# zkcrypto/jubjub

Measured on AMD Instinct MI355X. Metric: Jubjub scalar-muls/sec (varbase), higher is better.
Workload: dtype i32x9 (signed 29-bit limbs, v_mad_i64_i32 integer multiply-add)

## Files before the change

jubjub_amd/csrc/jj_field.h:

```cpp
#pragma once
#if !defined(JJ_EXPERIMENTS) && (defined(JJ_MUL_PIN) || defined(JJ_OPAQUE_MODE) || defined(JJ_VB_MINWAVES) || defined(JJ_VB_W) || defined(JJ_VB_PROBE_SHARED_READS) || \
    defined(JJ_FB_THREADS) || defined(JJ_FB_SINGLE_BUFFER) || defined(JJ_FBC_THREADS) || defined(JJ_FBC_SINGLE_BUFFER) || defined(JJ_FBC_PROBE) || \
    defined(JJ_MSM_SORT_UNROLL) || defined(JJ_MSM_P2_THREADS) || defined(JJ_MSM_ACC_MINBLOCKS))
#error "tuning / probe macros (JJ_VB_W, JJ_FB_THREADS, JJ_FBC_PROBE, ...) need -DJJ_EXPERIMENTS: the shipped library is built with the defaults"
#endif
#ifndef JJ_HOST_EMU
#include <hip/hip_runtime.h>
#endif
#include <stdint.h>
#include "jj_constants.h"

namespace jj {

#ifdef JJ_HOST_EMU
#define JJ_DEV inline
extern "C" void jj_emu_overflow(const char* what);
#define JJ_EMU_ACC_DECL __int128 acc_shadow = 0
#define JJ_EMU_ACC_MAD(x, y) do { acc_shadow += (__int128)(x) * (__int128)(y); if (acc_shadow != (__int128)acc) jj_emu_overflow("column accumulator"); } while (0)
#define JJ_EMU_ACC_SHIFT() do { acc_shadow >>= LB; } while (0)
#else
#define JJ_DEV __device__ __forceinline__
#define JJ_EMU_ACC_DECL
#define JJ_EMU_ACC_MAD(x, y)
#define JJ_EMU_ACC_SHIFT()
#endif

typedef int32_t i32;
typedef int64_t i64;

struct Fe {
  u32 l[NL];
};

#ifndef JJ_MUL_PIN
#define JJ_MUL_PIN 1
#endif
#ifndef JJ_OPAQUE_MODE
#define JJ_OPAQUE_MODE 1
#endif
template <class P, int PIN = JJ_MUL_PIN>
struct Field {
  static constexpr u32 PINV = (0u - P::NINV) & LMASK;

  static JJ_DEV Fe one() { Fe r; _Pragma("unroll") for (int i = 0; i < NL; i++) r.l[i] = P::ONE[i]; return r; }
  static JJ_DEV Fe zero() { Fe r; _Pragma("unroll") for (int i = 0; i < NL; i++) r.l[i] = 0; return r; }
  template <int N>
  static JJ_DEV Fe konst(const u32 (&c)[N]) { Fe r; _Pragma("unroll") for (int i = 0; i < NL; i++) r.l[i] = c[i]; return r; }

#ifdef JJ_HOST_EMU
#define JJ_OPAQUE(x) (x)
#else
#if JJ_OPAQUE_MODE == 1
static __device__ __forceinline__ u32 jj_opaque_asm(u32 x) { asm("" : "+v"(x)); return x; }
#define JJ_OPAQUE(x) jj_opaque_asm(x)
#else
#define JJ_OPAQUE(x) ((u32)__builtin_annotation((u32)(x), "jj"))
#endif
#endif
  template <bool SQUARE, bool DOUBLE, bool OPQ = true>
  static JJ_DEV Fe mul_fips(const Fe& a_in, const Fe& b_in) {
    i32 m[NL];
    i32 b2[NL], b4[NL];
    Fe a, b;
    _Pragma("unroll") for (int i = 0; i < NL; i++) {
      if constexpr (OPQ) { a.l[i] = JJ_OPAQUE(a_in.l[i]); b.l[i] = SQUARE ? a.l[i] : JJ_OPAQUE(b_in.l[i]); }
      else { a.l[i] = a_in.l[i]; b.l[i] = SQUARE ? a.l[i] : b_in.l[i]; }
    }
    if constexpr (SQUARE) {
      _Pragma("unroll") for (int i = 0; i < NL; i++) b2[i] = (i32)(a.l[i] << 1);
      if constexpr (DOUBLE) { _Pragma("unroll") for (int i = 0; i < NL; i++) b4[i] = (i32)(a.l[i] << 2); }
    }
    Fe r;
    i64 acc = 0;
    JJ_EMU_ACC_DECL;
#ifdef JJ_HOST_EMU
#define JJ_PIN(x)
#else
#define JJ_PIN(x) do { if constexpr (PIN == 1) x = __builtin_annotation(x, "jj"); } while (0)
#endif
#define JJ_MAD(x, y) do { acc += (i64)(i32)(x) * (i64)(i32)(y); JJ_EMU_ACC_MAD((i32)(x), (i32)(y)); JJ_PIN(acc); } while (0)
    _Pragma("unroll") for (int k = 0; k < 2 * NL - 1; k++) {
      _Pragma("unroll") for (int i = 0; i < NL; i++) {
        const int j = k - i;
        if (j < 0 || j >= NL) continue;
        if constexpr (SQUARE) {
          if (j > i) { if constexpr (DOUBLE) JJ_MAD(a.l[i], b4[j]); else JJ_MAD(a.l[i], b2[j]); }
          else if (j == i) { if constexpr (DOUBLE) JJ_MAD(a.l[i], b2[i]); else JJ_MAD(a.l[i], a.l[i]); }
        } else {
          JJ_MAD(a.l[i], b.l[j]);
        }
      }
      _Pragma("unroll") for (int i = 0; i < NL; i++) {
        const int j = k - i;
        if (i >= k || i >= NL || j < 1 || j >= NL) continue;
        JJ_MAD(m[i], -(i32)P::P[j]);
      }
      if (k < NL) {
        u32 mk;
        if constexpr (PINV == 1u) mk = (u32)acc & LMASK;
        else mk = ((u32)acc * PINV) & LMASK;
        m[k] = (i32)mk;
        if constexpr (P::P[0] != 1u) JJ_MAD(mk, -(i32)P::P[0]);
      } else {
        r.l[k - NL] = (u32)acc & LMASK;
      }
      acc >>= LB;
      JJ_EMU_ACC_SHIFT();
    }
    r.l[NL - 1] = (u32)acc;
#ifdef JJ_HOST_EMU
    if (acc != (i64)(i32)acc) jj_emu_overflow("top limb");
#endif
#undef JJ_MAD
#undef JJ_PIN
    return r;
  }
  static JJ_DEV Fe mul(const Fe& a, const Fe& b) { return mul_fips<false, false>(a, b); }
  static JJ_DEV Fe opaque(const Fe& a) { Fe r; _Pragma("unroll") for (int i = 0; i < NL; i++) r.l[i] = JJ_OPAQUE(a.l[i]); return r; }
  static JJ_DEV Fe mul_hidden(const Fe& a, const Fe& b) { return mul_fips<false, false, false>(a, b); }
  static JJ_DEV Fe sqr_hidden(const Fe& a) { return mul_fips<true, false, false>(a, a); }
  static JJ_DEV Fe sqr(const Fe& a) { return mul_fips<true, false>(a, a); }
  static JJ_DEV Fe sqr2(const Fe& a) { return mul_fips<true, true>(a, a); }

  static JJ_DEV Fe add(const Fe& a, const Fe& b) {
    Fe r; _Pragma("unroll") for (int i = 0; i < NL; i++) r.l[i] = a.l[i] + b.l[i]; return r;
  }
  static JJ_DEV Fe sub(const Fe& a, const Fe& b) {
    Fe r; _Pragma("unroll") for (int i = 0; i < NL; i++) r.l[i] = a.l[i] - b.l[i]; return r;
  }
  static JJ_DEV Fe neg(const Fe& a) {
    Fe r; _Pragma("unroll") for (int i = 0; i < NL; i++) r.l[i] = 0u - a.l[i]; return r;
  }
  static JJ_DEV Fe dbl(const Fe& a) { return add(a, a); }
  static JJ_DEV Fe dbl_sub(const Fe& a, const Fe& b) {
    Fe r; _Pragma("unroll") for (int i = 0; i < NL; i++) r.l[i] = (a.l[i] << 1) - b.l[i]; return r;
  }
  static JJ_DEV Fe cneg(const Fe& a, u32 mask) {
#ifndef JJ_HOST_EMU
    asm("" : "+v"(mask));
#endif
    Fe r; _Pragma("unroll") for (int i = 0; i < NL; i++) r.l[i] = (a.l[i] ^ mask) - mask; return r;
  }
  static JJ_DEV Fe carry(const Fe& a) {
    Fe r;
    r.l[0] = a.l[0] & LMASK;
    _Pragma("unroll") for (int i = 1; i < NL - 1; i++) r.l[i] = (a.l[i] & LMASK) + (u32)((i32)a.l[i - 1] >> LB);
    r.l[NL - 1] = a.l[NL - 1] + (u32)((i32)a.l[NL - 2] >> LB);
    return r;
  }
  static JJ_DEV Fe carry_full(const Fe& a) {
    Fe r; i32 c = 0;
    _Pragma("unroll") for (int i = 0; i < NL - 1; i++) { const i32 t = (i32)a.l[i] + c; r.l[i] = (u32)t & LMASK; c = t >> LB; }
    r.l[NL - 1] = a.l[NL - 1] + (u32)c;
    return r;
  }
  static JJ_DEV Fe select(const Fe& a, const Fe& b, u32 mask) {
#ifndef JJ_HOST_EMU
    asm("" : "+v"(mask));
#endif
    Fe r; _Pragma("unroll") for (int i = 0; i < NL; i++) r.l[i] = (b.l[i] & mask) | (a.l[i] & ~mask); return r;
  }

  static JJ_DEV Fe to_plain(const Fe& a) {
    Fe one_plain; _Pragma("unroll") for (int i = 0; i < NL; i++) one_plain.l[i] = (i == 0);
    const Fe t = mul(a, one_plain);
    const u32 negm = (u32)((i32)t.l[NL - 1] >> 31);
    Fe s; _Pragma("unroll") for (int i = 0; i < NL; i++) s.l[i] = t.l[i] + (P::P[i] & negm);
    return carry_full(s);
  }
  static JJ_DEV bool is_zero(const Fe& a) {
    Fe one_plain; _Pragma("unroll") for (int i = 0; i < NL; i++) one_plain.l[i] = (i == 0);
    const Fe t = mul(a, one_plain);
    u32 o0 = 0, o1 = 0;
    _Pragma("unroll") for (int i = 0; i < NL; i++) { o0 |= t.l[i]; o1 |= t.l[i] ^ P::NEGP_DIGITS[i]; }
    return o0 == 0 || o1 == 0;
  }
  static JJ_DEV bool eq(const Fe& a, const Fe& b) { return is_zero(sub(a, b)); }
  static JJ_DEV bool is_zero_product(const Fe& t) {
    u32 o0 = 0, o1 = 0;
    _Pragma("unroll") for (int i = 0; i < NL; i++) { o0 |= t.l[i]; o1 |= t.l[i] ^ P::NEGP_DIGITS[i]; }
    return o0 == 0 || o1 == 0;
  }
  static JJ_DEV Fe canon_plain_product(const Fe& a) {
    Fe w = a;
    _Pragma("unroll") for (int rep = 0; rep < 2; rep++) {
      const u32 negm = (u32)((i32)w.l[NL - 1] >> 31);
      Fe s; _Pragma("unroll") for (int i = 0; i < NL; i++) s.l[i] = w.l[i] + (P::P[i] & negm);
      w = carry_full(s);
    }
    return w;
  }
  static JJ_DEV Fe plain_one() { Fe r; _Pragma("unroll") for (int i = 0; i < NL; i++) r.l[i] = (i == 0); return r; }
  static JJ_DEV Fe canon(const Fe& a) {
    Fe w = mul(a, one());
    _Pragma("unroll") for (int rep = 0; rep < 2; rep++) {
      const u32 negm = (u32)((i32)w.l[NL - 1] >> 31);
      Fe s; _Pragma("unroll") for (int i = 0; i < NL; i++) s.l[i] = w.l[i] + (P::P[i] & negm);
      w = carry_full(s);
    }
    return w;
  }

  static JJ_DEV Fe unpack(const u32 (&w)[8]) {
    Fe r;
    _Pragma("unroll") for (int i = 0; i < NL; i++) {
      const int bit = LB * i, wi = bit >> 5, sh = bit & 31;
      u32 v = w[wi] >> sh;
      if (sh > 32 - LB && wi + 1 < 8) v |= w[wi + 1] << (32 - sh);
      r.l[i] = v & LMASK;
    }
    return r;
  }
  static JJ_DEV void pack(u32 (&w)[8], const Fe& a) {
    _Pragma("unroll") for (int wi = 0; wi < 8; wi++) {
      const int bit = 32 * wi, li = bit / LB, sh = bit % LB;
      u32 v = a.l[li] >> sh;
      const int got = LB - sh;
      if (got < 32 && li + 1 < NL) v |= a.l[li + 1] << got;
      if (got + LB < 32 && li + 2 < NL) v |= a.l[li + 2] << (got + LB);
      w[wi] = v;
    }
  }
  static JJ_DEV Fe from_words(const u32 (&w)[8]) { return mul(unpack(w), konst(P::R2)); }
  static JJ_DEV Fe from_words_checked(const u32 (&w)[8], bool& ok) {
    Fe x = unpack(w);
    i32 borrow = 0;
    _Pragma("unroll") for (int i = 0; i < NL; i++) { i32 t = (i32)x.l[i] - (i32)P::P[i] + borrow; borrow = t >> LB; }
    ok = (borrow != 0);
    return mul(x, konst(P::R2));
  }
  static JJ_DEV void to_words(u32 (&w)[8], const Fe& a) { pack(w, to_plain(a)); }
  static JJ_DEV Fe from_words_wide(const u32 (&lo)[8], const u32 (&hi)[8]) {
    return add(mul(unpack(lo), konst(P::R2)), mul(unpack(hi), konst(P::R2_256)));
  }

  struct PowProg { uint8_t nsq[80]; uint8_t idx[80]; int len; int first; };
  template <int NW>
  static constexpr PowProg make_prog(const u32 (&e)[NW]) {
    PowProg p{};
    bool started = false;
    int pend = 0, i = 32 * NW - 1;
    while (i >= 0) {
      if (!((e[i >> 5] >> (i & 31)) & 1u)) { if (started) pend++; i--; continue; }
      int j = i >= 3 ? i - 3 : 0;
      while (!((e[j >> 5] >> (j & 31)) & 1u)) j++;
      u32 val = 0;
      for (int b = i; b >= j; b--) val = (val << 1) | ((e[b >> 5] >> (b & 31)) & 1u);
      if (started) { p.nsq[p.len] = (uint8_t)(pend + (i - j + 1)); p.idx[p.len] = (uint8_t)(val >> 1); p.len++; }
      else { p.first = (int)(val >> 1); started = true; }
      pend = 0;
      i = j - 1;
    }
    if (pend) { p.nsq[p.len] = (uint8_t)pend; p.idx[p.len] = 255; p.len++; }
    return p;
  }
  template <int NW, const u32 (&E)[NW]>
  static JJ_DEV Fe pow_const(const Fe& a) {
    static constexpr PowProg prog = make_prog(E);
    const Fe a2 = sqr(a);
    const Fe t0 = a, t1 = mul(t0, a2), t2 = mul(t1, a2), t3 = mul(t2, a2), t4 = mul(t3, a2), t5 = mul(t4, a2), t6 = mul(t5, a2), t7 = mul(t6, a2);
    auto pick = [&](int idx) -> Fe {
      switch (idx) {
        case 0: return t0; case 1: return t1; case 2: return t2; case 3: return t3;
        case 4: return t4; case 5: return t5; case 6: return t6; default: return t7;
      }
    };
    Fe r = pick(prog.first);
    #pragma unroll 1
    for (int s = 0; s < prog.len; s++) {
      const int nsq = prog.nsq[s], idx = prog.idx[s];
      #pragma unroll 1
      for (int q = 0; q < nsq; q++) r = sqr(r);
      if (idx != 255) r = mul(r, pick(idx));
    }
    return r;
  }
  static JJ_DEV Fe invert(const Fe& a) { return pow_const<8, P::PM2>(a); }
};

typedef Field<FqP> Fq;
typedef Field<FrP> Fr;

}
```

jubjub_amd/csrc/jj_kernels.h:

```cpp
#pragma once
#include "jj_curve.h"
#include "jj_mont.h"

namespace jj {

static JJ_DEV void load8(u32 (&w)[8], const void* base, size_t idx) {
  const uint4* p = reinterpret_cast<const uint4*>(static_cast<const uint8_t*>(base) + idx * 32);
  const uint4 a = p[0], b = p[1];
  w[0] = a.x; w[1] = a.y; w[2] = a.z; w[3] = a.w; w[4] = b.x; w[5] = b.y; w[6] = b.z; w[7] = b.w;
}
static JJ_DEV void store8(void* base, size_t idx, const u32 (&w)[8]) {
  uint4* p = reinterpret_cast<uint4*>(static_cast<uint8_t*>(base) + idx * 32);
  p[0] = make_uint4(w[0], w[1], w[2], w[3]);
  p[1] = make_uint4(w[4], w[5], w[6], w[7]);
}
static JJ_DEV void zero8(u32 (&w)[8]) { _Pragma("unroll") for (int i = 0; i < 8; i++) w[i] = 0; }

struct SoA {
  u32* base;
  size_t n;
  JJ_DEV void put(int coord, size_t i, const Fe& a) const {
    _Pragma("unroll") for (int l = 0; l < NL; l++) base[((size_t)coord * NL + l) * n + i] = a.l[l];
  }
  JJ_DEV Fe get(int coord, size_t i) const {
// ... 60 lines not shown
  if (tid < 256) {
    Fe gam = Fq::konst(FqP::ROOT_POW2[24]);
    Fe p = Fq::one();
    for (int j = 0; j < tid; j++) p = Fq::mul(p, gam);
    dlog[Fq::to_plain(p).l[SQRT_KEY_LIMB] & 0xffffu] = (uint8_t)tid;
  } else if (tid < 256 + 1024) {
    const int i = (tid - 256) >> 8, k = (tid - 256) & 255;
    Fe base = Fq::konst(FqP::ROOT_OF_UNITY_INV);
    for (int j = 0; j < 8 * i; j++) base = Fq::sqr(base);
    Fe p = Fq::one();
    for (int j = 0; j < k; j++) p = Fq::mul(p, base);
    const Fe c = Fq::canon(p);
    _Pragma("unroll") for (int l = 0; l < NL; l++) npow[((size_t)i * 256 + k) * NL + l] = c.l[l];
  }
}
#endif

#ifdef JJ_KERNELS_BATCH
template <class P, int OP>
__global__ void __launch_bounds__(256) k_field_op(size_t n, const void* a, const void* b, void* out, uint8_t* okp, SqrtTables tabs) {
  typedef Field<P> F;
  const size_t i = (size_t)blockIdx.x * blockDim.x + threadIdx.x;
  if (i >= n) return;
  u32 wa[8], wb[8], wo[8];
  bool ok = true;
  Fe r;
  if constexpr (OP == OP_FROM_WIDE) {
    load8(wa, a, 2 * i); load8(wb, a, 2 * i + 1);
    r = F::from_words_wide(wa, wb);
  } else if constexpr (OP == OP_FROM_BYTES) {
    load8(wa, a, i);
    r = F::from_words_checked(wa, ok);
  } else {
    load8(wa, a, i);
    const Fe x = F::from_words(wa);
    if constexpr (OP == OP_ADD || OP == OP_SUB || OP == OP_MUL) {
      load8(wb, b, i);
      const Fe y = F::from_words(wb);
      if constexpr (OP == OP_ADD) r = F::add(x, y);
      if constexpr (OP == OP_SUB) r = F::sub(x, y);
      if constexpr (OP == OP_MUL) r = F::mul(x, y);
    }
    if constexpr (OP == OP_NEG) r = F::neg(x);
    if constexpr (OP == OP_SQUARE) r = F::sqr(x);
    if constexpr (OP == OP_DOUBLE) r = F::dbl(x);
    if constexpr (OP == OP_INVERT) { ok = !F::is_zero(x); r = F::invert(x); }
    if constexpr (OP == OP_SQRT) {
      if constexpr (P::PBITS == 255) r = fq_sqrt_fast(x, ok, tabs); else r = fr_sqrt(x, ok);
    }
  }
  F::to_words(wo, r);
  if (!ok) zero8(wo);
  store8(out, i, wo);
  if (okp) okp[i] = ok ? 1 : 0;
}
#endif

#ifdef JJ_KERNELS_BATCH
template <class P>
__global__ void __launch_bounds__(256) k_field_pow(size_t n, const void* a, const void* e, void* out) {
  typedef Field<P> F;
  const size_t i = (size_t)blockIdx.x * blockDim.x + threadIdx.x;
  if (i >= n) return;
  u32 wa[8], we[8], wo[8];
  load8(wa, a, i); load8(we, e, i);
  const Fe x = F::from_words(wa);
  Fe res = F::one();
  #pragma unroll 1
  for (int bit = 255; bit >= 0; bit--) {
    u32 word = we[0];
    _Pragma("unroll") for (int w = 1; w < 8; w++) word = ((bit >> 5) == w) ? we[w] : word;
    res = F::sqr(res);
    const Fe t = F::mul(res, x);
    res = F::select(res, t, 0u - ((word >> (bit & 31)) & 1u));
  }
  F::to_words(wo, res);
  store8(out, i, wo);
}
#endif

#ifdef JJ_KERNELS_BATCH
template <class P>
__global__ void __launch_bounds__(256) k_field_to_bits(size_t n, const void* a, void* out256) {
  typedef Field<P> F;
  const size_t i = (size_t)blockIdx.x * blockDim.x + threadIdx.x;
  if (i >= n) return;
  u32 wa[8], w[8];
  load8(wa, a, i);
  F::to_words(w, F::from_words(wa));
  uint4* o = reinterpret_cast<uint4*>(static_cast<uint8_t*>(out256) + i * 256);
  _Pragma("unroll") for (int v = 0; v < 16; v++) {
    const u32 h = (w[v >> 1] >> (16 * (v & 1))) & 0xffffu;
    u32 q[4];
    _Pragma("unroll") for (int k = 0; k < 4; k++) { const u32 nib = (h >> (4 * k)) & 15u; q[k] = (nib & 1u) | ((nib & 2u) << 7) | ((nib & 4u) << 14) | ((nib & 8u) << 21); }
    o[v] = make_uint4(q[0], q[1], q[2], q[3]);
  }
}
#endif

enum PointOp { PT_DOUBLE = 0, PT_ADD, PT_SUB, PT_NEG, PT_COFACTOR, PT_TO_NIELS,
               PT_IS_IDENTITY, PT_IS_SMALL_ORDER, PT_IS_ON_CURVE };

#ifdef JJ_KERNELS_BATCH
template <int OP>
__global__ void __launch_bounds__(256) k_point_op(size_t n, const void* p, const void* q, SoA ext, void* out) {
  const size_t i = (size_t)blockIdx.x * blockDim.x + threadIdx.x;
  if (i >= n) return;
  const Affine a = load_affine(p, i);
  Ext e = Curve::from_affine(a), r;
  if constexpr (OP == PT_DOUBLE) r = Curve::dbl(e);
  if constexpr (OP == PT_ADD) r = Curve::add<true>(e, Curve::to_niels(load_affine(q, i)));
  if constexpr (OP == PT_SUB) r = Curve::sub<true>(e, Curve::to_niels(load_affine(q, i)));
  if constexpr (OP == PT_NEG) r = Curve::neg(e);
  if constexpr (OP == PT_COFACTOR) r = Curve::mul_by_cofactor(e);
  if constexpr (OP <= PT_COFACTOR) { ext.put(0, i, r.u); ext.put(1, i, r.v); ext.put(2, i, r.z); }
  if constexpr (OP == PT_TO_NIELS) {
    const ANiels t = Curve::to_niels(a);
    u32 w[8];
    Fq::to_words(w, t.vpu); store8(out, 3 * i, w);
    Fq::to_words(w, t.vmu); store8(out, 3 * i + 1, w);
    Fq::to_words(w, t.t2d); store8(out, 3 * i + 2, w);
  }
  if constexpr (OP == PT_IS_IDENTITY) static_cast<uint8_t*>(out)[i] = Curve::is_identity(e);
  if constexpr (OP == PT_IS_SMALL_ORDER) static_cast<uint8_t*>(out)[i] = Curve::is_small_order(e);
  if constexpr (OP == PT_IS_ON_CURVE) static_cast<uint8_t*>(out)[i] = Curve::is_on_curve(a);
}
#endif

#ifdef JJ_KERNELS_BATCH
__global__ void __launch_bounds__(256) k_small_order_cofactor(size_t n, const void* pts, unsigned flags, SoA ext, uint8_t* ok) {
  const size_t i = (size_t)blockIdx.x * blockDim.x + threadIdx.x;
  if (i >= n) return;
  Ext e = Curve::dbl(Curve::dbl(Curve::from_affine(load_affine(pts, i))));
  if ((flags & 4u) && Fq::is_zero(e.u)) ok[i] = 0;
  if (flags & 8u) { e = Curve::dbl(e); ext.put(0, i, e.u); ext.put(1, i, e.v); ext.put(2, i, e.z); }
}
#endif

#ifdef JJ_KERNELS_BATCH
template <int CHUNK>
__global__ void __launch_bounds__(256) k_normalize(size_t n, size_t T, SoA ext, SoA scratch, void* out, int mode) {
  const size_t t = (size_t)blockIdx.x * blockDim.x + threadIdx.x;
  if (t >= T) return;
  Fe acc = Fq::one();
  #pragma unroll 1
  for (int j = 0; j < CHUNK; j++) {
    const size_t i = t + (size_t)j * T;
    if (i >= n) break;
    scratch.put(0, i, acc);
    const Fe z = ext.get(2, i);
    const u32 zz = Fq::is_zero_product(z) ? ~0u : 0u;
    acc = Fq::select(Fq::mul(acc, z), acc, zz);
  }
  Fe inv = Fq::mul(Fq::invert(acc), Fq::plain_one());
  #pragma unroll 1
  for (int j = CHUNK - 1; j >= 0; j--) {
    const size_t i = t + (size_t)j * T;
    if (i >= n) continue;
    const Fe z = ext.get(2, i);
    const u32 zz = Fq::is_zero_product(z) ? ~0u : 0u;
    const Fe zp = Fq::select(Fq::mul(inv, scratch.get(0, i)), Fq::zero(), zz);
    inv = Fq::select(Fq::mul(inv, z), inv, zz);
    u32 wu[8], wv[8];
    Fq::pack(wu, Fq::canon_plain_product(Fq::mul(ext.get(0, i), zp)));
    Fq::pack(wv, Fq::canon_plain_product(Fq::mul(ext.get(1, i), zp)));
    if (mode == 0) {
      store8(out, 2 * i, wu);
      store8(out, 2 * i + 1, wv);
    } else {
      wv[7] |= (wu[0] & 1u) << 31;
      store8(out, i, wv);
    }
  }
}
#endif

#ifdef JJ_KERNELS_BATCH
__global__ void __launch_bounds__(256) k_is_identity_ext(size_t n, SoA ext, uint8_t* out, int combine ) {
  const size_t i = (size_t)blockIdx.x * blockDim.x + threadIdx.x;
  if (i >= n) return;
  const bool id = Fq::is_zero(ext.get(0, i)) && Fq::eq(ext.get(1, i), ext.get(2, i));
  if (combine == 0) out[i] = id;
  else if (combine == 1) out[i] = out[i] & (id ? 1 : 0);
  else out[i] = out[i] & (id ? 0 : 1);
}
#endif

#ifdef JJ_KERNELS_BATCH
__global__ void __launch_bounds__(256) k_torsion_free(size_t n, const void* pts, uint8_t* out, int combine) {
  const size_t i = (size_t)blockIdx.x * blockDim.x + threadIdx.x;
  if (i >= n) return;
  const bool tf = Curve::is_torsion_free(load_affine(pts, i));
  out[i] = combine ? (out[i] & (tf ? 1 : 0)) : (tf ? 1 : 0);
}
#endif

#ifdef JJ_KERNELS_BATCH
__global__ void __launch_bounds__(256) k_ext160_to_soa(size_t n, const void* ext160, SoA ext) {
  const size_t i = (size_t)blockIdx.x * blockDim.x + threadIdx.x;
  if (i >= n) return;
  u32 w[8];
  _Pragma("unroll") for (int c = 0; c < 3; c++) { load8(w, ext160, 5 * i + c); ext.put(c, i, Fq::from_words(w)); }
}
#endif

#ifndef JJ_VB_MINWAVES
#define JJ_VB_MINWAVES 2
#endif
#ifndef JJ_VB_W
#define JJ_VB_W 5
#endif
constexpr int VB_W = JJ_VB_W;
constexpr int VB_TABLE = 1 << (VB_W - 1);
constexpr int VB_NWIN = (253 + VB_W - 1) / VB_W;
constexpr int ENIELS_WORDS = 4 * NL;

static JJ_DEV void store_eniels(u32* slot, const ENiels& n) {
  uint4* p = reinterpret_cast<uint4*>(slot);
  const Fe* c[4] = {&n.vpu, &n.vmu, &n.z2, &n.t2d};
  u32 w[ENIELS_WORDS];
  _Pragma("unroll") for (int k = 0; k < 4; k++) _Pragma("unroll") for (int l = 0; l < NL; l++) w[k * NL + l] = c[k]->l[l];
  _Pragma("unroll") for (int v = 0; v < ENIELS_WORDS / 4; v++) p[v] = make_uint4(w[4 * v], w[4 * v + 1], w[4 * v + 2], w[4 * v + 3]);
}
static JJ_DEV ENiels load_eniels(const u32* slot) {
  const uint4* p = reinterpret_cast<const uint4*>(slot);
  u32 w[ENIELS_WORDS];
  _Pragma("unroll") for (int v = 0; v < ENIELS_WORDS / 4; v++) { const uint4 x = p[v]; w[4 * v] = x.x; w[4 * v + 1] = x.y; w[4 * v + 2] = x.z; w[4 * v + 3] = x.w; }
  ENiels n;
  _Pragma("unroll") for (int l = 0; l < NL; l++) { n.vpu.l[l] = w[l]; n.vmu.l[l] = w[NL + l]; n.z2.l[l] = w[2 * NL + l]; n.t2d.l[l] = w[3 * NL + l]; }
  return n;
}
static JJ_DEV void recode_signed(u32 (&k)[8]) {
  k[7] &= 0x0fffffffu;
  u64 c = 0;
  _Pragma("unroll") for (int i = 0; i < 8; i++) {
    u32 rc = 0;
    _Pragma("unroll") for (int j = 0; j < VB_NWIN - 1; j++) { const int bit = VB_W * j + VB_W - 1; if ((bit >> 5) == i) rc |= 1u << (bit & 31); }
    const u64 t = (u64)k[i] + rc + c;
    k[i] = (u32)t; c = t >> 32;
  }
}
static JJ_DEV u32 vb_window(const u32 (&k)[8], int i) {
  const int bit = VB_W * i, wi = bit >> 5, sh = bit & 31;
  u32 lo = k[0], hi = k[1];
  _Pragma("unroll") for (int q = 1; q < 8; q++) { lo = (wi == q) ? k[q] : lo; hi = (wi == q) ? (q < 7 ? k[q + 1] : 0u) : hi; }
  const u64 both = ((u64)hi << 32) | lo;
  return (u32)(both >> sh) & ((1u << VB_W) - 1u);
}
constexpr int VB_SLOTS = VB_TABLE + 1;

static JJ_DEV Ext varbase_windowed(const Affine& P, u32 (&k)[8], u32* slot) {
#ifdef JJ_VB_PROBE_SHARED_READS
  const u32* rslot = slot - (size_t)threadIdx.x * (size_t)((1 << (JJ_VB_W - 1)) + 1) * (4 * NL);
#else
  const u32* rslot = slot;
#endif
  const ANiels pn = Curve::to_niels(P);
  Ext cur = Curve::from_affine(P);
  store_eniels(slot, Curve::eniels_identity());
  store_eniels(slot + ENIELS_WORDS, Curve::to_niels<true>(cur));
  #pragma unroll 1
  for (int j = 2; j <= VB_TABLE; j++) {
    cur = Curve::add<true>(cur, pn);
    store_eniels(slot + j * ENIELS_WORDS, Curve::to_niels<true>(cur));
  }
  recode_signed(k);
  u32 a = vb_window(k, VB_NWIN - 1), neg = 0;
  ENiels e = load_eniels(rslot + a * ENIELS_WORDS);
  Ext acc = Curve::identity();
  #pragma unroll 1
  for (int i = VB_NWIN - 1; i >= 0; i--) {
    const ENiels s = e;
    const u32 smask = neg ? ~0u : 0u;
    if (i > 0) {
      const int d = (int)vb_window(k, i - 1) - VB_TABLE;
      neg = d < 0; a = (u32)(d < 0 ? -d : d);
      e = load_eniels(rslot + a * ENIELS_WORDS);
    }
    acc = Curve::add_signed<true>(acc, s, smask);
    if (i > 0) {
      #pragma unroll 1
      for (int d = 0; d < (VB_W - 1) / 2; d++) acc = Curve::dbl(Curve::dbl(acc));
      if constexpr ((VB_W - 1) % 2) acc = Curve::dbl(acc);
      acc = Curve::dbl(acc);
    }
  }
  return acc;
}

static JJ_DEV bool next_wave_units(unsigned long long* cursor, size_t n, size_t& i) {
  unsigned long long base = 0;
  if ((threadIdx.x & 63u) == 0) base = atomicAdd(cursor, 64ull);
  const u32 lo = (u32)__builtin_amdgcn_readfirstlane((int)(u32)base), hi = (u32)__builtin_amdgcn_readfirstlane((int)(u32)(base >> 32));
  base = ((unsigned long long)hi << 32) | lo;
  i = (size_t)base + (threadIdx.x & 63u);
  return base < n;
}
#ifdef JJ_KERNELS_BATCH
template <bool FIVE, bool SHARED>
__global__ void __launch_bounds__(256, JJ_VB_MINWAVES) k_varbase(size_t n, const void* scalars, const void* points, u32* tables, SoA ext, unsigned long long* cursor) {
  const size_t gtid = (size_t)blockIdx.x * blockDim.x + threadIdx.x;
  u32* slot = tables + gtid * (size_t)(VB_SLOTS * ENIELS_WORDS);
  size_t i;
  #pragma unroll 1
  while (next_wave_units(cursor, n, i)) {
    if (i < n) {
      u32 k[8];
// ... 39 lines not shown
  const ENiels zero = Curve::eniels_identity();
  Ext acc = Curve::identity();
  #pragma unroll 1
  for (int i2 = 251; i2 >= 0; i2--) {
    u32 word = k[0];
    _Pragma("unroll") for (int w = 1; w < 8; w++) word = ((i2 >> 5) == w) ? k[w] : word;
    const u32 bit = (word >> (i2 & 31)) & 1u;
    acc = Curve::dbl(acc);
    acc = Curve::add<true>(acc, Curve::select(zero, pn, 0u - bit));
  }
  u32 w[8];
  Fq::to_words(w, acc.u); store8(out160, 5 * i, w);
  Fq::to_words(w, acc.v); store8(out160, 5 * i + 1, w);
  Fq::to_words(w, acc.z); store8(out160, 5 * i + 2, w);
  Fq::to_words(w, acc.t1); store8(out160, 5 * i + 3, w);
  Fq::to_words(w, acc.t2); store8(out160, 5 * i + 4, w);
}
#endif

constexpr int CT_NWIN = 127;
static JJ_DEV Ext varbase_ct(const Affine& P, u32 (&k)[8]) {
  const Ext p1 = Curve::from_affine(P);
  const ENiels e1 = Curve::to_niels<true>(p1);
  const ENiels e2 = Curve::to_niels<true>(Curve::dbl(p1));
  const ENiels idn = Curve::eniels_identity();
  k[7] &= 0x0fffffffu;
  {
    u64 cy = 0;
    _Pragma("unroll") for (int j = 0; j < 8; j++) { const u64 t = (u64)k[j] + (j < 7 ? 0xaaaaaaaau : 0x0aaaaaaau) + cy; k[j] = (u32)t; cy = t >> 32; }
  }
  const u32 top = (k[7] >> 28) & 1u;
  Ext acc = Curve::add<true>(Curve::identity(), Curve::select(idn, e1, 0u - top));
  u32 ks[8];
  _Pragma("unroll") for (int q = 7; q >= 1; q--) ks[q] = (k[q] << 4) | (k[q - 1] >> 28);
  ks[0] = k[0] << 4;
  #pragma unroll 1
  for (int i = CT_NWIN - 2; i >= 0; i--) {
    const int d = (int)(ks[7] >> 30) - 2;
    _Pragma("unroll") for (int q = 7; q >= 1; q--) ks[q] = (ks[q] << 2) | (ks[q - 1] >> 30);
    ks[0] <<= 2;
    const u32 sgn = (u32)(d >> 31);
    const u32 a = ((u32)d ^ sgn) - sgn;
    const ENiels e = Curve::select(Curve::select(idn, e1, 0u - (a & 1u)), e2, 0u - (a >> 1));
    acc = Curve::dbl(Curve::dbl(acc));
    acc = Curve::add_signed<true>(acc, e, sgn);
  }
  return acc;
}
#ifdef JJ_KERNELS_BATCH
__global__ void __launch_bounds__(256) k_varbase_ct(size_t n, const void* scalars, const void* points, SoA ext) {
  const size_t i = (size_t)blockIdx.x * blockDim.x + threadIdx.x;
  if (i >= n) return;
  u32 k[8];
  load8(k, scalars, i);
  const Affine P = load_affine(points, i);
  const Ext r = varbase_ct(P, k);
  ext.put(0, i, r.u); ext.put(1, i, r.v); ext.put(2, i, r.z);
}
#endif

constexpr int CT3_NWIN = 84;
constexpr int CT3_LDS_WORDS_PER_LANE = 2 * ENIELS_WORDS;
constexpr int CT3_LDS_BYTES_PER_BLOCK = 256 * CT3_LDS_WORDS_PER_LANE * 4;
static JJ_DEV u32 and_or(u32 a, u32 m, u32 c) { return (a & m) | c; }
static JJ_DEV Ext varbase_ct3(const Affine& P, u32 (&k)[8], uint4* slot , u32* kmem, size_t kstride) {
  const Ext p1 = Curve::from_affine(P);
  const ENiels e1 = Curve::to_niels<true>(p1);
  const Ext p2 = Curve::dbl(p1);
  const ENiels e2 = Curve::to_niels<true>(p2);
  {
    const Ext p3 = Curve::add<true>(p2, e1);
    const ENiels e3 = Curve::to_niels<true>(p3), e4 = Curve::to_niels<true>(Curve::dbl(p2));
    u32 w[CT3_LDS_WORDS_PER_LANE];
    _Pragma("unroll") for (int l = 0; l < NL; l++) {
      w[l] = e3.vpu.l[l]; w[NL + l] = e3.vmu.l[l]; w[2 * NL + l] = e3.z2.l[l]; w[3 * NL + l] = e3.t2d.l[l];
      w[ENIELS_WORDS + l] = e4.vpu.l[l]; w[ENIELS_WORDS + NL + l] = e4.vmu.l[l]; w[ENIELS_WORDS + 2 * NL + l] = e4.z2.l[l]; w[ENIELS_WORDS + 3 * NL + l] = e4.t2d.l[l];
    }
    _Pragma("unroll") for (int v = 0; v < CT3_LDS_WORDS_PER_LANE / 4; v++) slot[v * 64] = make_uint4(w[4 * v], w[4 * v + 1], w[4 * v + 2], w[4 * v + 3]);
  }
  k[7] &= 0x0fffffffu;
  {
    constexpr u32 RC[8] = {0x24924924u, 0x49249249u, 0x92492492u, 0x24924924u, 0x49249249u, 0x92492492u, 0x24924924u, 0x09249249u};
    u64 cy = 0;
    _Pragma("unroll") for (int j = 0; j < 8; j++) { const u64 t = (u64)k[j] + RC[j] + cy; k[j] = (u32)t; cy = t >> 32; }
  }
  const ENiels idn = Curve::eniels_identity();
  const u32 top = (k[7] >> 28) & 1u;
  Ext acc = Curve::add<true>(Curve::identity(), Curve::select(idn, e1, 0u - top));
  _Pragma("unroll") for (int q = 0; q < 8; q++) kmem[(size_t)q * kstride] = k[q];
  #pragma unroll 1
  for (int i = CT3_NWIN - 1; i >= 0; i--) {
    const int bit = 3 * i, wi = bit >> 5, sh = bit & 31;
    const u32 lo = kmem[(size_t)wi * kstride], hi = kmem[(size_t)(wi < 7 ? wi + 1 : 7) * kstride];
    const int d = (int)((u32)((((u64)hi << 32) | lo) >> sh) & 7u) - 4;
    const u32 sgn = (u32)(d >> 31);
    const u32 a = ((u32)d ^ sgn) - sgn;
    u32 m4 = 0u - (a >> 2), m3 = 0u - ((a >> 1) & a & 1u), m2 = 0u - ((a >> 1) & ~a & 1u), m1 = 0u - (a & ~(a >> 1) & 1u);
    asm("" : "+v"(m1), "+v"(m2), "+v"(m3), "+v"(m4));
    const u32 m0 = ~(m1 | m2 | m3 | m4);
    acc = Curve::dbl(Curve::dbl(acc));
    acc = Curve::dbl(acc);
    u32 sel[ENIELS_WORDS];
    _Pragma("unroll") for (int l = 0; l < NL; l++) {
      sel[l] = and_or(e1.vpu.l[l], m1, and_or(e2.vpu.l[l], m2, idn.vpu.l[l] & m0));
      sel[NL + l] = and_or(e1.vmu.l[l], m1, and_or(e2.vmu.l[l], m2, idn.vmu.l[l] & m0));
      sel[2 * NL + l] = and_or(e1.z2.l[l], m1, and_or(e2.z2.l[l], m2, idn.z2.l[l] & m0));
      sel[3 * NL + l] = and_or(e1.t2d.l[l], m1, e2.t2d.l[l] & m2);
    }
    _Pragma("unroll") for (int v = 0; v < ENIELS_WORDS / 4; v++) {
      const uint4 x3 = slot[v * 64], x4 = slot[(ENIELS_WORDS / 4 + v) * 64];
      sel[4 * v] = and_or(x3.x, m3, and_or(x4.x, m4, sel[4 * v]));
      sel[4 * v + 1] = and_or(x3.y, m3, and_or(x4.y, m4, sel[4 * v + 1]));
      sel[4 * v + 2] = and_or(x3.z, m3, and_or(x4.z, m4, sel[4 * v + 2]));
      sel[4 * v + 3] = and_or(x3.w, m3, and_or(x4.w, m4, sel[4 * v + 3]));
    }
    ENiels e;
    _Pragma("unroll") for (int l = 0; l < NL; l++) { e.vpu.l[l] = sel[l]; e.vmu.l[l] = sel[NL + l]; e.z2.l[l] = sel[2 * NL + l]; e.t2d.l[l] = sel[3 * NL + l]; }
    acc = Curve::add_signed<true>(acc, e, sgn);
  }
  return acc;
}
#ifdef JJ_KERNELS_BATCH
__global__ void __launch_bounds__(256, 2) k_varbase_ct3(size_t n, const void* scalars, const void* points, SoA ext) {
  extern __shared__ __attribute__((aligned(16))) uint4 ct3_lds[];
  const size_t i = (size_t)blockIdx.x * blockDim.x + threadIdx.x;
  uint4* slot = ct3_lds + (size_t)(threadIdx.x >> 6) * (CT3_LDS_WORDS_PER_LANE / 4) * 64 + (threadIdx.x & 63u);
  if (i >= n) return;
  u32 k[8];
  load8(k, scalars, i);
  const Affine P = load_affine(points, i);
  const Ext r = varbase_ct3(P, k, slot, ext.base + i, ext.n);
  ext.put(0, i, r.u); ext.put(1, i, r.v); ext.put(2, i, r.z);
}
#endif

#ifdef JJ_KERNELS_BATCH
__global__ void __launch_bounds__(256) k_varbase_mont_x1(size_t n, const void* points, SoA ext) {
  const size_t t = (size_t)blockIdx.x * blockDim.x + threadIdx.x;
  const size_t first = (t >> 6) * (size_t)(64 * MONT_X1_UNITS) + (t & 63u);
  if (first >= n) return;
  auto den_of = [&](size_t i, Fe& num) -> Fe {
    u32 wv[8];
    load8(wv, points, 2 * i + 1);
    return mont_x1_den(Fq::from_words(wv), num);
  };
  Fe acc = Fq::one(), num;
  #pragma unroll 1
  for (int s = 0; s < MONT_X1_UNITS; s++) {
    const size_t i = first + (size_t)s * 64;
    if (i >= n) break;
    ext.put(2, i, acc);
    acc = Fq::mul(acc, den_of(i, num));
  }
  Fe inv = Fq::invert(acc);
  #pragma unroll 1
  for (int s = MONT_X1_UNITS - 1; s >= 0; s--) {
    const size_t i = first + (size_t)s * 64;
    if (i >= n) continue;
    const Fe d = den_of(i, num);
    const Fe di = Fq::mul(inv, ext.get(2, i));
    inv = Fq::mul(inv, d);
    ext.put(2, i, Fq::mul(Fq::carry(num), di));
  }
}
__global__ void __launch_bounds__(256, 3) k_varbase_mont(size_t n, const void* scalars, const void* points, SoA ext) {
  const size_t i = (size_t)blockIdx.x * blockDim.x + threadIdx.x;
  if (i >= n) return;
  u32 k[8];
  load8(k, scalars, i);
  const Affine P = load_affine(points, i);
  const Fe x1 = ext.get(2, i);
  Fe u, v, z;
  varbase_mont(P, x1, k, u, v, z);
  ext.put(0, i, u); ext.put(1, i, v); ext.put(2, i, z);
}
#endif

constexpr int FB_W = 6;
constexpr int FB_NWIN = 42;
constexpr int FB_ENT = 33;
constexpr int FB_ENTRIES = FB_NWIN * FB_ENT + 1;
constexpr int ANIELS_WORDS = 28;
constexpr int GNIELS_WORDS = 32;
constexpr int FB_LDS_BYTES = FB_ENTRIES * ANIELS_WORDS * 4;

static JJ_DEV ANiels lds_aniels(const u32* e) {
  const uint4* p = reinterpret_cast<const uint4*>(e);
  u32 w[ANIELS_WORDS];
  _Pragma("unroll") for (int v = 0; v < ANIELS_WORDS / 4; v++) { const uint4 x = p[v]; w[4 * v] = x.x; w[4 * v + 1] = x.y; w[4 * v + 2] = x.z; w[4 * v + 3] = x.w; }
  ANiels n;
  _Pragma("unroll") for (int l = 0; l < NL; l++) { n.vpu.l[l] = w[l]; n.vmu.l[l] = w[NL + l]; n.t2d.l[l] = w[2 * NL + l]; }
  return n;
}
static JJ_DEV u32 window6(const u32 (&k)[8], int i) {
  const int bit = 6 * i, wi = bit >> 5, sh = bit & 31;
  u32 lo = k[0], hi = k[1];
  _Pragma("unroll") for (int w = 1; w < 8; w++) { lo = (wi == w) ? k[w] : lo; hi = (wi == w) ? (w < 7 ? k[w + 1] : 0u) : hi; }
  const u64 both = ((u64)hi << 32) | lo;
  return (u32)(both >> sh) & 63u;
}

static JJ_DEV Ext soa_ext(const SoA& s, size_t i);
#ifndef JJ_FB_THREADS
#define JJ_FB_THREADS 512
#endif
#ifndef JJ_FB_SINGLE_BUFFER
#define JJ_FB_SINGLE_BUFFER 0
#endif
constexpr int FB_THREADS = JJ_FB_THREADS;
#ifdef JJ_KERNELS_BATCH
template <bool CT>
__global__ void __launch_bounds__(FB_THREADS) k_fixedbase(size_t n, const void* scalars, const u32* table, SoA ext, int chain) {
  extern __shared__ __attribute__((aligned(16))) u32 lds[];
  {
    const uint4* src = reinterpret_cast<const uint4*>(table);
    uint4* dst = reinterpret_cast<uint4*>(lds);
    for (int v = threadIdx.x; v < FB_LDS_BYTES / 16; v += blockDim.x) dst[v] = src[v];
  }
  __syncthreads();
  const size_t T = (size_t)gridDim.x * blockDim.x;
  const u32 lane = threadIdx.x & 63u;
  const size_t n_round = (n + 63) & ~(size_t)63;
  #pragma unroll 1
  for (size_t idx = (size_t)blockIdx.x * blockDim.x + threadIdx.x; idx < n_round; idx += T) {
    const bool live = idx < n;
    u32 k[8];
    if (live) load8(k, scalars, idx); else zero8(k);
    k[7] &= 0x0fffffffu;
    {
      u64 c = 0;
      _Pragma("unroll") for (int i = 0; i < 8; i++) { const u64 t = (u64)k[i] + RECODE6[i] + c; k[i] = (u32)t; c = t >> 32; }
    }
    const u32 top = (k[7] >> 28) & 1u;
    const ANiels idn = Curve::aniels_identity();
    Ext acc = Curve::identity();
    if ((chain & 1) && live) acc = soa_ext(ext, idx);
    acc = Curve::add<true>(acc, Curve::select(idn, lds_aniels(lds + (size_t)(FB_NWIN * FB_ENT) * ANIELS_WORDS), 0u - top));
    u32 ks[8];
    _Pragma("unroll") for (int q = 7; q >= 1; q--) ks[q] = (k[q] << 4) | (k[q - 1] >> 28);
    ks[0] = k[0] << 4;
    auto next_digit = [&](u32& j, u32& negmask) {
      const int d = (int)(ks[7] >> 26) - 32;
      _Pragma("unroll") for (int q = 7; q >= 1; q--) ks[q] = (ks[q] << 6) | (ks[q - 1] >> 26);
      ks[0] <<= 6;
      const u32 sgn = (u32)(d >> 31);
      j = ((u32)d ^ sgn) - sgn;
      negmask = sgn;
    };
    auto fetch = [&](int i, u32 j) -> ANiels {
      if constexpr (CT) {
        const ANiels mine = lds_aniels(lds + ((size_t)i * FB_ENT + (lane < (u32)FB_ENT ? lane : lane - (u32)FB_ENT)) * ANIELS_WORDS);
        const int src = (int)(j << 2);
        ANiels e;
        _Pragma("unroll") for (int l = 0; l < NL; l++) {
          e.vpu.l[l] = (u32)__builtin_amdgcn_ds_bpermute(src, (int)mine.vpu.l[l]);
          e.vmu.l[l] = (u32)__builtin_amdgcn_ds_bpermute(src, (int)mine.vmu.l[l]);
          e.t2d.l[l] = (u32)__builtin_amdgcn_ds_bpermute(src, (int)mine.t2d.l[l]);
        }
        return e;
      } else {
        return lds_aniels(lds + ((size_t)i * FB_ENT + j) * ANIELS_WORDS);
      }
    };
    static_assert(FB_NWIN % 2 == 0, "the window loop is unrolled by two");
    u32 j, neg0, neg1;
#if JJ_FB_SINGLE_BUFFER
    #pragma unroll 1
    for (int i = FB_NWIN - 1; i >= 0; i--) {
      next_digit(j, neg0);
      const ANiels e = fetch(i, j);
      acc = Curve::add_signed<true>(acc, e, neg0);
    }
    (void)neg1;
#else
    next_digit(j, neg0);
    ANiels e0 = fetch(FB_NWIN - 1, j), e1;
    #pragma unroll 1
    for (int i = FB_NWIN - 1; i >= 1; i -= 2) {
      next_digit(j, neg1);
      e1 = fetch(i - 1, j);
      acc = Curve::add_signed<true>(acc, e0, neg0);
      if (i > 1) { next_digit(j, neg0); e0 = fetch(i - 2, j); }
      acc = Curve::add_signed<true>(acc, e1, neg1);
    }
#endif
    if (live) {
      ext.put(0, idx, acc.u); ext.put(1, idx, acc.v); ext.put(2, idx, acc.z);
      if (chain & 2) { ext.put(3, idx, Fq::carry(acc.t1)); ext.put(4, idx, Fq::carry(acc.t2)); }
    }
  }
}
#endif
constexpr int FBC_TEETH = 8, FBC_SPACING = 32, FBC_BLOCKS = 8, FBC_COLS = 4;
constexpr int FBC_TENT = 128;
constexpr int FBC_TABLES = FBC_BLOCKS + 2;
constexpr int FBC_ENTRIES = FBC_TABLES * FBC_TENT;
constexpr int FBC_LDS_BYTES = FBC_ENTRIES * ANIELS_WORDS * 4;
#ifndef JJ_FBC_THREADS
#define JJ_FBC_THREADS 768
#endif
#ifndef JJ_FBC_SINGLE_BUFFER
#define JJ_FBC_SINGLE_BUFFER 1
#endif
constexpr int FBC_THREADS = JJ_FBC_THREADS;
#ifdef JJ_KERNELS_BATCH
template <bool CT>
__global__ void __launch_bounds__(FBC_THREADS) k_fixedbase_comb(size_t n, const void* scalars, const u32* table, SoA ext, int chain) {
// ... 623 lines not shown
```

jubjub_amd/csrc/jj_mont.h:

```cpp
#pragma once
#include "jj_curve.h"

namespace jj {

struct MontK {
  static constexpr u32 TWO_A[9] = {0x1fa7aa4fu, 0x02c2ad87u, 0x1bae6c40u, 0x0936fbd9u, 0x11652c16u, 0x13ce2c45u, 0x10c0760eu, 0x117bd639u, 0x006b8a64u};
  static constexpr u32 TWO_B[9] = {0x005856cdu, 0x1d3d4998u, 0x0fd54cbfu, 0x1aafac22u, 0x08f9624fu, 0x00a72b80u, 0x1fa2daa0u, 0x16c980a5u, 0x00301b3bu};
  static constexpr u32 NEG_ONE[9] = {0x00000047u, 0x1ffffdc8u, 0x02e0ee3fu, 0x10f9a9ffu, 0x0e97a399u, 0x151d55f1u, 0x1c18d42bu, 0x021155b7u, 0x0026e968u};
};
constexpr int MONT_NBITS = 252;
constexpr i32 MONT_A24 = 10240;
constexpr i32 MONT_A24_QMUL = 0x58549745;
constexpr int MONT_X1_UNITS = 16;

static JJ_DEV Fe mont_a24(const Fe& e) {
  const i32 qd = (i32)(((i64)(i32)e.l[NL - 1] * (i64)MONT_A24_QMUL) >> 40);
  i64 t[NL];
  _Pragma("unroll") for (int i = 0; i < NL; i++) t[i] = (i64)(i32)e.l[i] * (i64)MONT_A24 - (i64)qd * (i64)FqP::P[i];
  Fe r;
  r.l[0] = (u32)t[0] & LMASK;
  _Pragma("unroll") for (int i = 1; i < NL; i++) r.l[i] = (i < NL - 1 ? ((u32)t[i] & LMASK) : (u32)t[i]) + (u32)(t[i - 1] >> LB);
#ifdef JJ_HOST_EMU
  if (t[NL - 1] + (t[NL - 2] >> LB) != (i64)(i32)r.l[NL - 1]) jj_emu_overflow("a24 top limb");
#endif
  return r;
}

static JJ_DEV void mont_xdbladd(const Fe& ox1, Fe& x2, Fe& z2, Fe& x3, Fe& z3) {
  typedef Fq F;
  const Fe oa = F::opaque(F::carry(F::add(x2, z2)));
  const Fe ob = F::opaque(F::sub(x2, z2));
  const Fe aa = F::sqr_hidden(oa), bb = F::sqr_hidden(ob);
  const Fe da = F::mul_hidden(F::opaque(F::sub(x3, z3)), oa);
  const Fe cb = F::mul_hidden(F::opaque(F::add(x3, z3)), ob);
  const Fe e = F::sub(aa, bb);
  const Fe w = F::add(aa, mont_a24(e));
  x3 = F::sqr(F::carry(F::add(da, cb)));
  z3 = F::mul_hidden(ox1, F::opaque(F::sqr(F::sub(da, cb))));
  z2 = F::mul(e, w);
  x2 = F::mul(aa, bb);
}

static JJ_DEV Fe mont_x1_den(const Fe& v, Fe& num) {
  num = Fq::add(Fq::one(), v);
  const Fe d = Fq::sub(Fq::one(), v);
  return Fq::select(d, Fq::one(), 0u - (u32)Fq::is_zero(d));
}

static JJ_DEV u32 mont_zero_mask(const Fe& t) { return 0u - (u32)Fq::is_zero_product(t); }

static JJ_DEV void varbase_mont(const Affine& P, const Fe& x1, const u32 (&k_in)[8], Fe& ou, Fe& ov, Fe& oz) {
  typedef Fq F;
  u32 k[8];
  _Pragma("unroll") for (int q = 0; q < 8; q++) k[q] = k_in[q];
  k[7] &= 0x0fffffffu;
  u32 g[8];
  _Pragma("unroll") for (int q = 0; q < 8; q++) g[q] = k[q] ^ ((k[q] >> 1) | (q < 7 ? k[q + 1] << 31 : 0u));
  _Pragma("unroll") for (int q = 7; q >= 1; q--) g[q] = (g[q] << 4) | (g[q - 1] >> 28);
  g[0] <<= 4;
  const Fe ox1 = F::opaque(x1);
  Fe x2 = F::one(), z2 = F::zero(), x3 = x1, z3 = F::one();
  #pragma unroll 1
  for (int i = 0; i < MONT_NBITS; i++) {
    u32 sw = (u32)((i32)g[7] >> 31);
    _Pragma("unroll") for (int q = 7; q >= 1; q--) g[q] = (g[q] << 1) | (g[q - 1] >> 31);
    g[0] <<= 1;
    const Fe sx2 = F::select(x2, x3, sw), sx3 = F::select(x3, x2, sw);
    const Fe sz2 = F::select(z2, z3, sw), sz3 = F::select(z3, z2, sw);
    x2 = sx2; x3 = sx3; z2 = sz2; z3 = sz3;
    mont_xdbladd(ox1, x2, z2, x3, z3);
  }
  const u32 last = 0u - (k[0] & 1u);
  const Fe xq = F::select(x2, x3, last), zq = F::select(z2, z3, last);
  const Fe xp = F::select(x3, x2, last), zp = F::select(z3, z2, last);

  const Fe v1 = F::mul(x1, zq);
  const Fe v3 = F::mul(F::sqr(F::sub(xq, v1)), xp);
  const Fe t = F::mul(F::konst(MontK::TWO_A), zq);
  const Fe v4 = F::add(F::mul(x1, xq), zq);
  Fe v2 = F::mul(F::carry(F::add(F::add(xq, v1), t)), v4);
  v2 = F::mul(F::sub(v2, F::mul(t, zq)), zp);
  const Fe Y = F::mul(P.u, F::sub(v2, v3));
  const Fe w = F::mul(F::mul(F::mul(F::konst(MontK::TWO_B), x1), zq), zp);
  const Fe X = F::mul(w, xq), Z = F::mul(w, zq);
  const Fe xpz = F::add(X, Z);
  Fe U = F::mul(X, xpz), V = F::mul(Y, F::sub(X, Z)), W = F::mul(Y, xpz);

  const Fe one = F::one(), zero = F::zero(), negone = F::konst(MontK::NEG_ONE);
  const u32 zp0 = mont_zero_mask(zp), zq0 = mont_zero_mask(zq), xq0 = mont_zero_mask(xq) & ~zq0;
  const u32 x10 = mont_zero_mask(x1);
  const u32 ident = 0u - (u32)F::is_zero(F::sub(P.v, one));
  const u32 odd = last;
  U = F::select(U, F::mul(P.u, negone), zp0); V = F::select(V, P.v, zp0); W = F::select(W, one, zp0);
  U = F::select(U, zero, xq0); V = F::select(V, negone, xq0); W = F::select(W, one, xq0);
  const u32 to_id = zq0 | (x10 & ~odd) | ident;
  const u32 to_t2 = x10 & odd & ~ident;
  U = F::select(U, zero, to_id | to_t2); V = F::select(F::select(V, one, to_id), negone, to_t2); W = F::select(W, one, to_id | to_t2);
  ou = U; ov = V; oz = W;
}

}
```

Baseline: 76.53 million.

## Use divsteps inversion and fold the ladder swap into the differential add

Adds a constant-time Bernstein-Yang divsteps field inversion on 30-bit signed limbs and uses it in place of Fermat exponentiation in the batch-normalize and Montgomery x1 kernels. The Montgomery ladder step no longer swaps the x/z pairs. It computes sums and differences for both points and selects only the pair that feeds the doubling, using the fact that the differential-add cross products are symmetric under the swap. Both changes aim to cut inversion cost and per-bit select overhead. In exchange they add code complexity, register pressure and new overflow-bound reasoning.

Result: faster. 78.22 million (median of 6 runs) (+2.2%).

```diff
diff --git a/jubjub_amd/csrc/jj_field.h b/jubjub_amd/csrc/jj_field.h
--- a/jubjub_amd/csrc/jj_field.h
+++ b/jubjub_amd/csrc/jj_field.h
@@ -38,6 +38,28 @@
 #ifndef JJ_OPAQUE_MODE
 #define JJ_OPAQUE_MODE 1
 #endif
+constexpr int DS_LB = 30;
+constexpr u32 DS_MASK = 0x3fffffffu;
+constexpr int DS_BATCHES = ((49 * 256 + 57) / 17 + DS_LB - 1) / DS_LB;
+struct DsMod { int32_t p[NL]; u32 pinv; };
+template <class P>
+constexpr DsMod make_dsmod() {
+  DsMod m{};
+  for (int i = 0; i < NL; i++) {
+    u32 v = 0;
+    for (int b = 0; b < DS_LB; b++) {
+      const int bit = DS_LB * i + b, li = bit / LB, lo = bit % LB;
+      if (li < NL) v |= ((P::P[li] >> lo) & 1u) << b;
+    }
+    m.p[i] = (int32_t)v;
+  }
+  const u32 p0 = (u32)m.p[0] | ((u32)m.p[1] << DS_LB);
+  u32 x = p0;
+  for (int k = 0; k < 5; k++) x *= 2u - p0 * x;
+  m.pinv = x & DS_MASK;
+  return m;
+}
+
 template <class P, int PIN = JJ_MUL_PIN>
 struct Field {
   static constexpr u32 PINV = (0u - P::NINV) & LMASK;
@@ -276,6 +298,120 @@
     return r;
   }
   static JJ_DEV Fe invert(const Fe& a) { return pow_const<8, P::PM2>(a); }
+
+#ifdef JJ_HOST_EMU
+#define JJ_DS_ACC(name) i64 name = 0; __int128 name##_shadow = 0
+#define JJ_DS_MAD(name, x, y) do { name += (i64)(i32)(x) * (i64)(i32)(y); name##_shadow += (__int128)(i32)(x) * (__int128)(i32)(y); if (name##_shadow != (__int128)name) jj_emu_overflow("divsteps accumulator"); } while (0)
+#define JJ_DS_SHIFT(name) do { name >>= DS_LB; name##_shadow >>= DS_LB; } while (0)
+  static bool ds_in_range(const i32 (&d)[NL], const DsMod& M) {
+    i64 lo = 0, hi = 0;
+    for (int i = 0; i < NL; i++) { lo = (lo >> DS_LB) + d[i] + 2 * (i64)M.p[i]; hi = (hi >> DS_LB) + d[i] - (i64)M.p[i]; }
+    bool lo_zero = true; i64 c = 0;
+    for (int i = 0; i < NL; i++) { c = (c >> DS_LB) + d[i] + 2 * (i64)M.p[i]; if (i < NL - 1 ? (c & DS_MASK) != 0 : c != 0) lo_zero = false; }
+    return lo >= 0 && !lo_zero && hi < 0;
+  }
+#else
+#define JJ_DS_ACC(name) i64 name = 0
+#define JJ_DS_MAD(name, x, y) name += (i64)(i32)(x) * (i64)(i32)(y)
+#define JJ_DS_SHIFT(name) name >>= DS_LB
+#endif
+  static JJ_DEV Fe invert_divsteps(const Fe& a) {
+    constexpr DsMod M = make_dsmod<P>();
+    u32 w[8];
+    pack(w, to_plain(a));
+    i32 f[NL], g[NL], d[NL], e[NL];
+    _Pragma("unroll") for (int i = 0; i < NL; i++) {
+      const int bit = DS_LB * i, wi = bit >> 5, sh = bit & 31;
+      u32 v = w[wi] >> sh;
+      if (sh > 32 - DS_LB && wi + 1 < 8) v |= w[wi + 1] << (32 - sh);
+      g[i] = (i32)(v & DS_MASK);
+      f[i] = M.p[i]; d[i] = 0; e[i] = (i == 0);
+    }
+    u32 eta = ~0u;
+    #pragma unroll 1
+    for (int batch = 0; batch < DS_BATCHES; batch++) {
+      u32 u = 1, v = 0, q = 0, r = 1, fl = (u32)f[0], gl = (u32)g[0];
+      _Pragma("unroll") for (int s = 0; s < DS_LB; s++) {
+        u32 c1 = (u32)((i32)eta >> 31);
+        const u32 c2 = 0u - (gl & 1u);
+        gl += ((fl ^ c1) - c1) & c2; q += ((u ^ c1) - c1) & c2; r += ((v ^ c1) - c1) & c2;
+        c1 &= c2;
+        eta = (eta ^ c1) - (c1 + 1u);
+        fl += gl & c1; u += q & c1; v += r & c1;
+        gl >>= 1; u <<= 1; v <<= 1;
+      }
+      u = JJ_OPAQUE(u); v = JJ_OPAQUE(v); q = JJ_OPAQUE(q); r = JJ_OPAQUE(r);
+      {
+        const u32 sd = (u32)(d[NL - 1] >> 31), se = (u32)(e[NL - 1] >> 31);
+        u32 md = (u & sd) + (v & se), me = (q & sd) + (r & se);
+        JJ_DS_ACC(cd); JJ_DS_ACC(ce);
+        const i32 d0 = (i32)JJ_OPAQUE((u32)d[0]), e0 = (i32)JJ_OPAQUE((u32)e[0]);
+        JJ_DS_MAD(cd, u, d0); JJ_DS_MAD(cd, v, e0);
+        JJ_DS_MAD(ce, q, d0); JJ_DS_MAD(ce, r, e0);
+        md -= (M.pinv * (u32)cd + md) & DS_MASK;
+        me -= (M.pinv * (u32)ce + me) & DS_MASK;
+        md = JJ_OPAQUE(md); me = JJ_OPAQUE(me);
+        JJ_DS_MAD(cd, M.p[0], md); JJ_DS_MAD(ce, M.p[0], me);
+#ifdef JJ_HOST_EMU
+        if (((u32)cd | (u32)ce) & DS_MASK) jj_emu_overflow("divsteps: low limb of the (d, e) update not cleared");
+#endif
+        JJ_DS_SHIFT(cd); JJ_DS_SHIFT(ce);
+        _Pragma("unroll") for (int i = 1; i < NL; i++) {
+          const i32 di = (i32)JJ_OPAQUE((u32)d[i]), ei = (i32)JJ_OPAQUE((u32)e[i]);
+          JJ_DS_MAD(cd, u, di); JJ_DS_MAD(cd, v, ei); JJ_DS_MAD(cd, M.p[i], md);
+          JJ_DS_MAD(ce, q, di); JJ_DS_MAD(ce, r, ei); JJ_DS_MAD(ce, M.p[i], me);
+          d[i - 1] = (i32)((u32)cd & DS_MASK); e[i - 1] = (i32)((u32)ce & DS_MASK);
+          JJ_DS_SHIFT(cd); JJ_DS_SHIFT(ce);
+        }
+        d[NL - 1] = (i32)cd; e[NL - 1] = (i32)ce;
+#ifdef JJ_HOST_EMU
+        if (cd != (i64)(i32)cd || ce != (i64)(i32)ce) jj_emu_overflow("divsteps: top limb of d, e");
+        if (!ds_in_range(d, M) || !ds_in_range(e, M)) jj_emu_overflow("divsteps: d or e left (-2p, p)");
+#endif
+      }
+      {
+        JJ_DS_ACC(cf); JJ_DS_ACC(cg);
+        const i32 f0 = (i32)JJ_OPAQUE((u32)f[0]), g0 = (i32)JJ_OPAQUE((u32)g[0]);
+        JJ_DS_MAD(cf, u, f0); JJ_DS_MAD(cf, v, g0);
+        JJ_DS_MAD(cg, q, f0); JJ_DS_MAD(cg, r, g0);
+#ifdef JJ_HOST_EMU
+        if (((u32)cf | (u32)cg) & DS_MASK) jj_emu_overflow("divsteps: low limb of the (f, g) update not zero");
+#endif
+        JJ_DS_SHIFT(cf); JJ_DS_SHIFT(cg);
+        _Pragma("unroll") for (int i = 1; i < NL; i++) {
+          const i32 fi = (i32)JJ_OPAQUE((u32)f[i]), gi = (i32)JJ_OPAQUE((u32)g[i]);
+          JJ_DS_MAD(cf, u, fi); JJ_DS_MAD(cf, v, gi);
+          JJ_DS_MAD(cg, q, fi); JJ_DS_MAD(cg, r, gi);
+          f[i - 1] = (i32)((u32)cf & DS_MASK); g[i - 1] = (i32)((u32)cg & DS_MASK);
+          JJ_DS_SHIFT(cf); JJ_DS_SHIFT(cg);
+        }
+        f[NL - 1] = (i32)cf; g[NL - 1] = (i32)cg;
+#ifdef JJ_HOST_EMU
+        if (cf != (i64)(i32)cf || cg != (i64)(i32)cg) jj_emu_overflow("divsteps: top limb of f, g");
+#endif
+      }
+    }
+#ifdef JJ_HOST_EMU
+    { u32 o = 0; for (int i = 0; i < NL; i++) o |= (u32)g[i]; if (o) jj_emu_overflow("divsteps: g != 0 after the last batch"); }
+#endif
+    const u32 sf = (u32)(f[NL - 1] >> 31);
+    u32 n[NL];
+    i32 c = 0;
+    _Pragma("unroll") for (int i = 0; i < NL - 1; i++) { const i32 t = (i32)(((u32)d[i] ^ sf) - sf) + c; n[i] = (u32)t & DS_MASK; c = t >> DS_LB; }
+    n[NL - 1] = (((u32)d[NL - 1] ^ sf) - sf) + (u32)c;
+    Fe x;
+    _Pragma("unroll") for (int i = 0; i < NL - 1; i++) {
+      const int bit = LB * i, j = bit / DS_LB, sh = bit % DS_LB;
+      u32 t = n[j] >> sh;
+      if (DS_LB - sh < LB) t |= n[j + 1] << (DS_LB - sh);
+      x.l[i] = t & LMASK;
+    }
+    x.l[NL - 1] = (n[NL - 2] >> (LB * (NL - 1) - DS_LB * (NL - 2))) + (n[NL - 1] << (DS_LB * (NL - 1) - LB * (NL - 1)));
+    return mul(x, konst(P::R2));
+  }
+#undef JJ_DS_ACC
+#undef JJ_DS_MAD
+#undef JJ_DS_SHIFT
 };
 
 typedef Field<FqP> Fq;
diff --git a/jubjub_amd/csrc/jj_kernels.h b/jubjub_amd/csrc/jj_kernels.h
--- a/jubjub_amd/csrc/jj_kernels.h
+++ b/jubjub_amd/csrc/jj_kernels.h
@@ -236,7 +236,7 @@
     const u32 zz = Fq::is_zero_product(z) ? ~0u : 0u;
     acc = Fq::select(Fq::mul(acc, z), acc, zz);
   }
-  Fe inv = Fq::mul(Fq::invert(acc), Fq::plain_one());
+  Fe inv = Fq::mul(Fq::invert_divsteps(acc), Fq::plain_one());
   #pragma unroll 1
   for (int j = CHUNK - 1; j >= 0; j--) {
     const size_t i = t + (size_t)j * T;
@@ -582,7 +582,7 @@
     ext.put(2, i, acc);
     acc = Fq::mul(acc, den_of(i, num));
   }
-  Fe inv = Fq::invert(acc);
+  Fe inv = Fq::invert_divsteps(acc);
   #pragma unroll 1
   for (int s = MONT_X1_UNITS - 1; s >= 0; s--) {
     const size_t i = first + (size_t)s * 64;
diff --git a/jubjub_amd/csrc/jj_mont.h b/jubjub_amd/csrc/jj_mont.h
--- a/jubjub_amd/csrc/jj_mont.h
+++ b/jubjub_amd/csrc/jj_mont.h
@@ -26,13 +26,13 @@
   return r;
 }
 
-static JJ_DEV void mont_xdbladd(const Fe& ox1, Fe& x2, Fe& z2, Fe& x3, Fe& z3) {
+static JJ_DEV void mont_xdbladd(const Fe& ox1, u32 sw, Fe& x2, Fe& z2, Fe& x3, Fe& z3) {
   typedef Fq F;
-  const Fe oa = F::opaque(F::carry(F::add(x2, z2)));
-  const Fe ob = F::opaque(F::sub(x2, z2));
+  const Fe s2 = F::opaque(F::add(x2, z2)), d2 = F::opaque(F::sub(x2, z2)), s3 = F::opaque(F::add(x3, z3)), d3 = F::opaque(F::sub(x3, z3));
+  const Fe oa = F::opaque(F::carry(F::opaque(F::select(s2, s3, sw))));
+  const Fe ob = F::opaque(F::select(d2, d3, sw));
+  const Fe da = F::mul_hidden(d3, s2), cb = F::mul_hidden(s3, d2);
   const Fe aa = F::sqr_hidden(oa), bb = F::sqr_hidden(ob);
-  const Fe da = F::mul_hidden(F::opaque(F::sub(x3, z3)), oa);
-  const Fe cb = F::mul_hidden(F::opaque(F::add(x3, z3)), ob);
   const Fe e = F::sub(aa, bb);
   const Fe w = F::add(aa, mont_a24(e));
   x3 = F::sqr(F::carry(F::add(da, cb)));
@@ -65,10 +65,7 @@
     u32 sw = (u32)((i32)g[7] >> 31);
     _Pragma("unroll") for (int q = 7; q >= 1; q--) g[q] = (g[q] << 1) | (g[q - 1] >> 31);
     g[0] <<= 1;
-    const Fe sx2 = F::select(x2, x3, sw), sx3 = F::select(x3, x2, sw);
-    const Fe sz2 = F::select(z2, z3, sw), sz3 = F::select(z3, z2, sw);
-    x2 = sx2; x3 = sx3; z2 = sz2; z3 = sz3;
-    mont_xdbladd(ox1, x2, z2, x3, z3);
+    mont_xdbladd(ox1, sw, x2, z2, x3, z3);
   }
   const u32 last = 0u - (k[0] & 1u);
   const Fe xq = F::select(x2, x3, last), zq = F::select(z2, z3, last);
```
